# secondlaw-ai/skyrim

Measured on AMD Instinct MI355X. Metric: 6-h forecast steps/sec on 721x1440 state, 1/2/4/8 MI355X; per-channel max rel-err vs ref, higher is better.
Workload: dtype f16; 1 GPU; Pangu 6-h autoregressive rollout, 721x1440x69 state (13 levels x 5 vars + 4 surface), random-init weights (64 M params), state resident in HBM, 1 ensemble membe; parallelism=single GPU, members=1, finite=True, rounding=compensated, term_plan=0x66f

## Files before the change

skyrim_amd/csrc/api.hip:

```cpp
#include <cstdio>
#include <cstdlib>
#include <cstring>
#include <string>
#include <type_traits>
#include <vector>

#include "../../include/skyrim_pangu.h"
#include "launchers.h"

using namespace skp;

namespace {

constexpr int kDepths[4] = {2, 6, 6, 2};
constexpr int kBiasRows = 3312;

int pad_to(int n, int mult, int* front, int pad_mode) {
    const int padded = (n + mult - 1) / mult * mult;
    if (front) *front = pad_mode == SKPANGU_PAD_CENTRE ? (padded - n) / 2 : 0;
    return padded;
}

bool make_geom(const skpangu_config& c, Geom& g) {
    if (c.n_lat < 8 || c.n_lon <= 0 || c.n_lon % 96 != 0) return false;
// ... 127 lines not shown
        }
        prof_cat[prof_used] = cat;
        (void)hipEventRecord(prof_ev[prof_used], s);
        ++prof_used;
    }
    void profile(bool on) override { prof_on = on; prof_used = 0; }
    ~Engine() override { for (hipEvent_t e : prof_ev) (void)hipEventDestroy(e); }
    hipError_t profile_read(skpangu_stage_stat* out, int cap, int* n) override {
        static const char* names_split[C_COUNT] = {"embed", "qkv_r0", "attn_r0", "proj_r0", "fc1_r0", "fc2_r0", "qkv_r1", "attn_r1",
                                                   "proj_r1", "fc1_r1", "fc2_r1", "downsample", "upsample", "recover"};
        static const char* names_block[C_COUNT] = {"embed", "qkv_r0", "attn_r0", "proj_r0", "proj_mlp_r0", "fc2_r0", "qkv_r1", "attn_r1",
                                                   "proj_r1", "proj_mlp_r1", "fc2_r1", "downsample", "upsample", "recover"};
        const char* const* names = fused_block ? names_block : names_split;
        double ms[C_COUNT] = {0}; int cnt[C_COUNT] = {0};
        if (prof_used > 0) {
            hipError_t e = hipEventSynchronize(prof_ev[prof_used - 1]);
            if (e != hipSuccess) return e;
        }
        for (size_t i = 0; i + 1 < prof_used; ++i) {
            if (prof_cat[i] < 0) continue;
            float t = 0.f;
            hipError_t e = hipEventElapsedTime(&t, prof_ev[i], prof_ev[i + 1]);
            if (e != hipSuccess) return e;
            ms[prof_cat[i]] += t; cnt[prof_cat[i]]++;
        }
        const double sa = 2.0 * NPL, hw = (double)g.H1 * g.W1, NA_ = P::NA;
        double fl[C_COUNT], by[C_COUNT];
        for (int r = 0; r < 2; ++r) {
            const double C = r == 0 ? 192 : 384, mw = g.mwin[r], nt = g.ntok[r], heads = C / 32, wb = 2.0 * NW;
            const int o = r == 0 ? 0 : 5;
            fl[C_QKV0 + o] = 2 * mw * C * 3 * C;      by[C_QKV0 + o] = nt * C * 2 * NA_ + 3 * mw * C * 2 + 3 * C * C * wb;
            fl[C_ATTN0 + o] = g.nwin[r] * heads * 4.0 * 144 * 144 * 32;
            by[C_ATTN0 + o] = 3 * mw * C * 2 + mw * C * sa + (double)g.types[r] * heads * 3456 * 2;
            fl[C_PROJ0 + o] = 2 * mw * C * C;          by[C_PROJ0 + o] = mw * C * sa + 2 * nt * C * 4 + C * C * wb;
            fl[C_FC1_0 + o] = 2 * nt * C * 4 * C;      by[C_FC1_0 + o] = nt * C * 2 * NA_ + nt * 4 * C * sa + 4 * C * C * wb;
            fl[C_FC2_0 + o] = 2 * nt * C * 4 * C;      by[C_FC2_0 + o] = nt * 4 * C * sa + 2 * nt * C * 4 + 4 * C * C * wb;
            const int nblk = kDepths[r == 0 ? 0 : 1] + kDepths[r == 0 ? 3 : 2];
            const int nqa = r == 0 ? (qa_fused(0) ? kDepths[0] : 0) + (qa_fused(3) ? kDepths[3] : 0)
                                   : (qa_fused(1) ? kDepths[1] : 0) + (qa_fused(2) ? kDepths[2] : 0);
            if (nqa > 0) {
                const double qa_fl = fl[C_ATTN0 + o] + fl[C_QKV0 + o];
                const double qa_by = nt * C * 2 + mw * C * sa + 3 * C * C * wb + (double)g.types[r] * heads * 3456 * 2;
                fl[C_ATTN0 + o] = nqa == nblk ? qa_fl : (nqa * qa_fl + (nblk - nqa) * fl[C_ATTN0 + o]) / nblk;
                by[C_ATTN0 + o] = nqa == nblk ? qa_by : (nqa * qa_by + (nblk - nqa) * by[C_ATTN0 + o]) / nblk;
            }
            if (fused_block) {
                fl[C_FC1_0 + o] = 4 * nt * C * 4 * C;  by[C_FC1_0 + o] = 2 * nt * C * 4 + 8 * C * C * wb;
                fl[C_FC1_0 + o] += 2 * mw * C * C;     by[C_FC1_0 + o] += nt * C * sa + C * C * wb;
            }
        }
        fl[C_EMBED] = 2 * hw * 112 * 192 + 2 * 7 * hw * 160 * 192; by[C_EMBED] = (69.0 + 3) * g.n_lat * g.n_lon * 4 + g.ntok[0] * 192.0 * 4;
        fl[C_DOWN] = 2.0 * g.ntok[1] * 768 * 384;                   by[C_DOWN] = g.ntok[0] * 192.0 * 4 + g.ntok[1] * 384.0 * 4;
        fl[C_UP] = 2.0 * g.ntok[1] * 384 * 768 + 2.0 * g.ntok[0] * 192 * 192;
        by[C_UP] = g.ntok[1] * 384.0 * 4 + 2 * g.ntok[0] * 192.0 * sa + g.ntok[0] * 192.0 * 4;
        fl[C_RECOVER] = 2 * hw * 384 * 64 + 2 * 7 * hw * 384 * 160; by[C_RECOVER] = 2 * g.ntok[0] * 192.0 * 4 + 69.0 * g.n_lat * g.n_lon * 4;
        int k = 0;
        for (int c = 0; c < C_COUNT && k < cap; ++c, ++k) {
            std::memset(&out[k], 0, sizeof(out[k]));
            std::strncpy(out[k].name, names[c], sizeof(out[k].name) - 1);
            out[k].launches = cnt[c]; out[k].total_ms = ms[c]; out[k].flops = fl[c]; out[k].bytes = by[c];
        }
        *n = k;
        prof_used = 0;
        return hipSuccess;
    }

    LinW<T> take_lin(Arena& a, int N, int ldd) {
        LinW<T> l;
        const long long plane = (long long)N * ldd;
        l.w = a.take<T>((size_t)plane * NW);
        l.plane = plane; l.ldw = ldd;
        return l;
    }

    void plan_prepared(char* base) {
        Arena a{base, 0};
        w.mean = a.take<float>(69); w.std = a.take<float>(69); w.istd = a.take<float>(69);
        w.masks = a.take<float>((size_t)3 * g.n_lat * g.n_lon);
        w.embed_u = take_lin(a, 192, 160); w.embed_s = take_lin(a, 192, 128);
        w.embed_u_b = a.take<float>(192); w.embed_s_b = a.take<float>(192);
        int b = 0;
        for (int layer = 0; layer < 4; ++layer) {
            const int c = layer_dim(layer), heads = layer_heads(layer), res = layer_res(layer);
            for (int i = 0; i < kDepths[layer]; ++i, ++b) {
                BlockW<T>& bw = w.blk[b];
                bw.qkv = take_lin(a, 3 * c, c); bw.proj = take_lin(a, c, c);
                bw.fc1 = take_lin(a, 4 * c, c); bw.fc2 = take_lin(a, c, 4 * c);
                const bool t2 = two_term(layer);
                bw.w1f = fused_block && !t2 ? a.take<T>((size_t)8 * c * c) : nullptr;
                bw.w2f = fused_block && !t2 ? a.take<T>((size_t)8 * c * c) : nullptr;
                bw.projf = fused_block && !t2 ? a.take<T>((size_t)2 * c * c) : nullptr;
                bw.projh = t2 ? a.take<T>((size_t)c * c) : nullptr;
                bw.w1h = t2 ? a.take<T>((size_t)4 * c * c) : nullptr;
                bw.w2h = t2 ? a.take<T>((size_t)4 * c * c) : nullptr;
                bw.qkvf = rt_qkv && !qkv_one(layer) ? a.take<T>((size_t)6 * c * c) : nullptr;
                bw.qkvh = qkv_one(layer) ? a.take<T>((size_t)3 * c * c) : nullptr;
                bw.qkv_b = a.take<float>(3 * c); bw.proj_b = a.take<float>(c);
                bw.fc1_b = a.take<float>(4 * c); bw.fc2_b = a.take<float>(c);
                bw.n1_g = a.take<float>(c); bw.n1_b = a.take<float>(c);
                bw.n2_g = a.take<float>(c); bw.n2_b = a.take<float>(c);
                bias_elems[b] = (size_t)g.types[res] * heads * 3456;
                bw.bias_cmp = a.take<f16>(bias_elems[b]);
            }
        }
        w.down_g = a.take<float>(768); w.down_b = a.take<float>(768);
        w.down = take_lin(a, 384, 768);
        w.up1 = take_lin(a, 768, 384); w.up2 = take_lin(a, 192, 192);
        w.up_g = a.take<float>(192); w.up_b = a.take<float>(192);
        w.rec_u = take_lin(a, 160, 384); w.rec_s = take_lin(a, 64, 384);
        w.rec_u_b = a.take<float>(5); w.rec_s_b = a.take<float>(4);
        for (int r = 0; r < 2; ++r)
            for (int roll = 0; roll < 2; ++roll) { w.widx[r][roll] = a.take<int>(g.mwin[r]); w.winv[r][roll] = a.take<int>(g.ntok[r]); }
        zrow = a.take<T>(4096);
        qkv_w_tmp = a.take<float>((size_t)3 * 384 * 384); qkv_b_tmp = a.take<float>(3 * 384);
        cal_sum = a.take<float>(4 * 384);
        prep_bytes = (a.off + 255) / 256 * 256;
    }

    void plan_workspace(char* base) {
        Arena a{base, 0};
        const size_t n0 = (size_t)g.ntok[0] * 192, n1 = (size_t)g.ntok[1] * 384;
        wk.xs_plane[0] = (long long)n0; wk.xs_plane[1] = (long long)n1;
        wk.X1s = a.take<T>(n0 * 2); wk.X2s = a.take<T>(n1 * 2); wk.X4s = a.take<T>(n0 * 2);
        const size_t m0 = (size_t)g.mwin[0] * 192, m1 = (size_t)g.mwin[1] * 384;
        q_elems = m0 > m1 ? m0 : m1;
        wk.qkv_plane = (long long)q_elems;
        wk.q = a.take<f16>(q_elems); wk.k = a.take<f16>(q_elems); wk.vt = a.take<f16>(q_elems);
        ao_elems = q_elems;
        wk.ao_plane = (long long)ao_elems;
        wk.ao = a.take<T>(ao_elems * NPL);
        const size_t h0 = (size_t)g.ntok[0] * 768, h1 = (size_t)g.ntok[1] * 1536;
        hid_elems = h0 > h1 ? h0 : h1;
        wk.hid_plane = (long long)hid_elems;
        wk.hid = a.take<T>(hid_elems * NPL);
        wk.u_plane = (long long)n0;
        wk.u = a.take<T>(n0 * NPL);
        wk.stats = a.take<float2>((size_t)g.ntok[1]);
        ws_bytes = (a.off + 255) / 256 * 256;
    }

    explicit Engine(const Geom& geom, int qkv_a1 = 0, int mlp_mode = 0, int term_plan = 0) : g(geom) {
        fused_qa = getenv("SKP_SPLIT_ATTN") == nullptr;
        fused_block = mlp_mode == 0;
        rt_qkv = (std::is_same<P, PrecF16x3>::value && qkv_a1 && mlp_mode == 0);
        plan2 = (std::is_same<P, PrecF16x3>::value && fused_block) ? term_plan : 0;
        wk.qkv_a1 = qkv_a1;
        params = build_params(g, nullptr);
        plan_prepared(nullptr);
        plan_workspace(nullptr);
    }
    size_t prepared_bytes() const override { return prep_bytes; }
    size_t workspace_bytes() const override { return ws_bytes; }
    void bind(char* prepared, char* workspace) override { plan_prepared(prepared); plan_workspace(workspace); }

    const float* P_(const float* master, const std::string& name) const {
        for (const Param& p : params)
            if (p.name == name) return master + p.offset;
        return nullptr;
    }
    hipError_t copyf(const float* dst, const float* src, size_t n, hipStream_t s) {
        return hipMemcpyAsync(const_cast<float*>(dst), src, n * sizeof(float), hipMemcpyDeviceToDevice, s);
    }
    hipError_t lin(const LinW<T>& l, const float* src, int N, int K, long long sn, long long sk, hipStream_t s, int blocked = 1, int perm = 1) {
        return prep_weight<T, NW>(src, const_cast<T*>(l.w), l.plane, N, K, l.ldw, sn, sk, blocked, perm, s);
    }

#define CK(x) do { hipError_t e_ = (x); if (e_ != hipSuccess) return e_; } while (0)

    hipError_t prepare(const float* m, hipStream_t s) override {
        wk.zrow = zrow;
        CK(hipMemsetAsync(zrow, 0, 4096 * sizeof(T), s));
        CK(copyf(w.mean, P_(m, "norm.mean"), 69, s));
        CK(copyf(w.std, P_(m, "norm.std"), 69, s));
        CK(prep_reciprocal(P_(m, "norm.std"), const_cast<float*>(w.istd), 69, s));
        CK(copyf(w.masks, P_(m, "const_masks"), (size_t)3 * g.n_lat * g.n_lon, s));
        CK(lin(w.embed_u, P_(m, "embed.conv.weight"), 192, 160, 160, 1, s, 0));
        CK(lin(w.embed_s, P_(m, "embed.conv_surface.weight"), 192, 112, 112, 1, s, 0));
        CK(copyf(w.embed_u_b, P_(m, "embed.conv.bias"), 192, s));
        CK(copyf(w.embed_s_b, P_(m, "embed.conv_surface.bias"), 192, s));
        int b = 0;
        for (int layer = 0; layer < 4; ++layer) {
            const int c = layer_dim(layer), heads = layer_heads(layer), res = layer_res(layer);
            for (int i = 0; i < kDepths[layer]; ++i, ++b) {
                const std::string p = "layer" + std::to_string(layer + 1) + ".block" + std::to_string(i) + ".";
                const BlockW<T>& bw = w.blk[b];
                const float *qkv_w = P_(m, p + "attn.qkv.weight"), *qkv_bias = P_(m, p + "attn.qkv.bias");
                if (g.qkv_order) {
                    CK(prep_qkv_rows(qkv_w, qkv_bias, qkv_w_tmp, qkv_b_tmp, c, heads, s));
                    qkv_w = qkv_w_tmp; qkv_bias = qkv_b_tmp;
                }
                CK(lin(bw.qkv, qkv_w, 3 * c, c, c, 1, s));
                CK(lin(bw.proj, P_(m, p + "attn.proj.weight"), c, c, c, 1, s));
                CK(lin(bw.fc1, P_(m, p + "mlp.fc1.weight"), 4 * c, c, c, 1, s));
                CK(lin(bw.fc2, P_(m, p + "mlp.fc2.weight"), c, 4 * c, 4 * c, 1, s));
                if (bw.projf) CK(prep_rowtile_weights<T>(P_(m, p + "attn.proj.weight"), const_cast<T*>(bw.projf), c, c, s));
                if (bw.qkvf) CK(prep_rowtile_weights<T>(qkv_w, const_cast<T*>(bw.qkvf), 3 * c, c, s));
                if (bw.qkvh) CK(prep_rowtile_weights<T>(qkv_w, const_cast<T*>(bw.qkvh), 3 * c, c, s, 1));
                if (bw.w1f) CK(prep_mlp_weights<T>(P_(m, p + "mlp.fc1.weight"), P_(m, p + "mlp.fc2.weight"), const_cast<T*>(bw.w1f), const_cast<T*>(bw.w2f), c, s));
                if (bw.projh) {
                    CK(prep_rowtile_weights<T>(P_(m, p + "attn.proj.weight"), const_cast<T*>(bw.projh), c, c, s, 1));
                    CK(prep_mlp_weights<T>(P_(m, p + "mlp.fc1.weight"), P_(m, p + "mlp.fc2.weight"), const_cast<T*>(bw.w1h), const_cast<T*>(bw.w2h), c, s, 1));
                }
                CK(copyf(bw.qkv_b, qkv_bias, 3 * c, s));
                CK(copyf(bw.proj_b, P_(m, p + "attn.proj.bias"), c, s));
                CK(copyf(bw.fc1_b, P_(m, p + "mlp.fc1.bias"), 4 * c, s));
                CK(copyf(bw.fc2_b, P_(m, p + "mlp.fc2.bias"), c, s));
                CK(copyf(bw.n1_g, P_(m, p + "norm1.weight"), c, s));
                CK(copyf(bw.n1_b, P_(m, p + "norm1.bias"), c, s));
                CK(copyf(bw.n2_g, P_(m, p + "norm2.weight"), c, s));
                CK(copyf(bw.n2_b, P_(m, p + "norm2.bias"), c, s));
                CK(prep_bias_compact(P_(m, p + "attn.bias_table"), const_cast<f16*>(bw.bias_cmp), g.types[res], heads, g.nH[res], (i & 1) ? g.roll_sign : 0, g.mask_value, s, g.bias_transposed));
            }
        }
        CK(copyf(w.down_g, P_(m, "down.norm.weight"), 768, s));
        CK(copyf(w.down_b, P_(m, "down.norm.bias"), 768, s));
        CK(lin(w.down, P_(m, "down.linear.weight"), 384, 768, 768, 1, s, 0));
        CK(lin(w.up1, P_(m, "up.linear1.weight"), 768, 384, 384, 1, s));
        CK(lin(w.up2, P_(m, "up.linear2.weight"), 192, 192, 192, 1, s));
        CK(copyf(w.up_g, P_(m, "up.norm.weight"), 192, s));
        CK(copyf(w.up_b, P_(m, "up.norm.bias"), 192, s));
        CK(lin(w.rec_u, P_(m, "recover.conv.weight"), 160, 384, 1, 160, s, 1, 0));
        CK(lin(w.rec_s, P_(m, "recover.conv_surface.weight"), 64, 384, 1, 64, s, 1, 0));
        CK(copyf(w.rec_u_b, P_(m, "recover.conv.bias"), 5, s));
        CK(copyf(w.rec_s_b, P_(m, "recover.conv_surface.bias"), 4, s));
        const int H[2] = {g.H1, g.H2}, W[2] = {g.W1, g.W2};
        for (int r = 0; r < 2; ++r)
            for (int roll = 0; roll < 2; ++roll)
            {
                CK(prep_window_index(const_cast<int*>(w.widx[r][roll]), g.Z, H[r], W[r], g.Hp[r], g.top[r], roll ? g.roll_sign : 0, s, g.surface_last));
                CK(prep_window_inverse(w.widx[r][roll], g.mwin[r], const_cast<int*>(w.winv[r][roll]), s));
            }
        return hipSuccess;
    }

    static int block_index(int layer0, int i) {
        int b = 0;
        for (int l = 0; l < layer0; ++l) b += kDepths[l];
        return b + i;
    }

    hipError_t block_planes(int layer0, int i, T* xs, hipStream_t s) {
        const int res = layer_res(layer0), C = layer_dim(layer0), heads = layer_heads(layer0);
        const BlockW<T>& bw = w.blk[block_index(layer0, i)];
        const int* widx = w.widx[res][i & 1];
        const int o = res == 0 ? 0 : 5;
        bool fused = false;
        if constexpr (std::is_same<P, PrecF16x3>::value) {
            if (qa_fused(layer0)) {
                mark(C_ATTN0 + o, s);
                CK(op_qkv_attention(g, bw, widx, res, xs, wk, s, block_one(layer0) ? 1 : 2));
                fused = true;
            }
        }
        if (!fused) {
            mark(C_QKV0 + o, s);
            if constexpr (std::is_same<P, PrecF16x3>::value) {
                if (rt_qkv) CK(op_qkv_rowtile(g, bw, widx, res, xs, wk, s));
                else CK((op_qkv<P>(g, bw, widx, res, xs, wk, s)));
            } else {
                CK((op_qkv<P>(g, bw, widx, res, xs, wk, s)));
            }
            mark(C_ATTN0 + o, s);
            AttnArgs<P> a{wk.q, wk.k, wk.vt, bw.bias_cmp, wk.ao, wk.ao_plane, C, g.nwin[res], g.nW[res], heads};
            a.out_planes = block_one(layer0) ? 1 : 0;
            CK(launch_attention<P>(a, s));
        }
        if constexpr (std::is_same<P, PrecF16x3>::value) {
            if (two_term(layer0)) {
                mark(C_FC1_0 + o, s);
                CK(op_proj_mlp2(g, bw, w.winv[res][i & 1], res, xs, wk, s, block_one(layer0)));
                mark(-1, s);
// ... 91 lines not shown
            for (int i = 0; i < kDepths[layer]; ++i, ++b) {
                const int C = layer_dim(layer), heads = layer_heads(layer);
                const std::string p = "layer" + std::to_string(layer + 1) + ".block" + std::to_string(i) + ".";
                const BlockW<T>& bw = w.blk[b];
                const float *qkv_w = P_(m, p + "attn.qkv.weight"), *qkv_bias = P_(m, p + "attn.qkv.bias");
                if (g.qkv_order) { CK(prep_qkv_rows(qkv_w, qkv_bias, qkv_w_tmp, qkv_b_tmp, C, heads, s)); qkv_bias = qkv_b_tmp; }
                CK(copyf(bw.qkv_b, qkv_bias, 3 * C, s));
                CK(copyf(bw.proj_b, P_(m, p + "attn.proj.bias"), C, s));
                CK(copyf(bw.fc1_b, P_(m, p + "mlp.fc1.bias"), 4 * C, s));
                CK(copyf(bw.fc2_b, P_(m, p + "mlp.fc2.bias"), C, s));
            }
        return hipSuccess;
    }
    hipError_t calibrate(const float* m, const float* in, hipStream_t s) override {
        if (plan2 == 0) return hipSuccess;
        if (!in) return master_biases(m, s);
        if constexpr (std::is_same<P, PrecF16x3>::value) {
            CK((op_embed<P>(g, w, in, wk.X1s, wk, s)));
            for (int i = 0; i < kDepths[0]; ++i) CK(calib_block(m, 0, i, wk.X1s, s));
            CK((op_down<P>(g, w, wk.X1s, wk.X2s, wk, s)));
            for (int i = 0; i < kDepths[1]; ++i) CK(calib_block(m, 1, i, wk.X2s, s));
            for (int i = 0; i < kDepths[2]; ++i) CK(calib_block(m, 2, i, wk.X2s, s));
            CK((op_up<P>(g, w, wk.X2s, wk.X4s, wk, s)));
            for (int i = 0; i < kDepths[3]; ++i) CK(calib_block(m, 3, i, wk.X4s, s));
        }
        return hipSuccess;
    }

    hipError_t step(const float* in, float* out, hipStream_t s) override {
        mark(C_EMBED, s);
        CK((op_embed<P>(g, w, in, wk.X1s, wk, s)));
        for (int i = 0; i < kDepths[0]; ++i) CK(block_planes(0, i, wk.X1s, s));
        mark(C_DOWN, s);
        CK((op_down<P>(g, w, wk.X1s, wk.X2s, wk, s)));
        for (int i = 0; i < kDepths[1]; ++i) CK(block_planes(1, i, wk.X2s, s));
        for (int i = 0; i < kDepths[2]; ++i) CK(block_planes(2, i, wk.X2s, s));
        mark(C_UP, s);
        CK((op_up<P>(g, w, wk.X2s, wk.X4s, wk, s)));
        for (int i = 0; i < kDepths[3]; ++i) CK(block_planes(3, i, wk.X4s, s));
        mark(C_RECOVER, s);
        CK((op_recover<P>(g, w, wk.X1s, wk.X4s, out, wk, s)));
        mark(-1, s);
        return hipSuccess;
    }
#undef CK

    bool debug(const std::string& n, void** p, size_t* bytes) override {
        auto set = [&](const void* ptr, size_t b) { *p = const_cast<void*>(ptr); *bytes = b; return true; };
        if (n == "q") return set(wk.q, q_elems * sizeof(f16));
        if (n == "k") return set(wk.k, q_elems * sizeof(f16));
        if (n == "vt") return set(wk.vt, q_elems * sizeof(f16));
        if (n == "ao") return set(wk.ao, ao_elems * NPL * sizeof(T));
        if (n == "hid") return set(wk.hid, hid_elems * NPL * sizeof(T));
        if (n == "u") return set(wk.u, (size_t)g.ntok[0] * 192 * NPL * sizeof(T));
        if (n == "x1") return set(wk.X1s, (size_t)g.ntok[0] * 192 * 2 * sizeof(T));
        if (n == "x2") return set(wk.X2s, (size_t)g.ntok[1] * 384 * 2 * sizeof(T));
        if (n == "x4") return set(wk.X4s, (size_t)g.ntok[0] * 192 * 2 * sizeof(T));
        if (n.rfind("widx", 0) == 0 && n.size() == 6) {
            const int r = n[4] - '0', roll = n[5] - '0';
            if (r < 0 || r > 1 || roll < 0 || roll > 1) return false;
            return set(w.widx[r][roll], (size_t)g.mwin[r] * 4);
        }
        if (n.rfind("bias_exp", 0) == 0) {
            const int b = atoi(n.c_str() + 8);
            if (b < 0 || b > 15) return false;
            return set(w.blk[b].bias_cmp, bias_elems[b] * sizeof(f16));
        }
        return false;
    }
};

IEngine* make_engine(const skpangu_config& cfg, const Geom& g) {
    switch (cfg.precision) {
        case SKPANGU_PREC_BF16X3: return new Engine<PrecBF16x3>(g, 0, cfg.mlp_mode);
        case SKPANGU_PREC_F16X3: return new Engine<PrecF16x3>(g, 0, cfg.mlp_mode, cfg.term_plan);
        case SKPANGU_PREC_F16X3_Q: return new Engine<PrecF16x3>(g, 1, cfg.mlp_mode, cfg.term_plan);
        default: return nullptr;
    }
}

}

struct skpangu_ctx {
    skpangu_config cfg;
    Geom g;
    IEngine* eng;
    bool prepared;
};

extern "C" {

int skpangu_abi_version(void) { return SKPANGU_ABI_VERSION; }

const char* skpangu_error_string(int code) {
    switch (code) {
        case 0: return "success";
        case SKPANGU_E_ARG: return "bad argument or unsupported geometry";
        case SKPANGU_E_SIZE: return "caller buffer too small";
        case SKPANGU_E_STATE: return "context not prepared";
        case SKPANGU_E_NOTFOUND: return "not found";
        default: return code > 0 ? hipGetErrorString((hipError_t)code) : "unknown error";
    }
}

int skpangu_query_sizes(const skpangu_config* cfg, skpangu_sizes* out) {
    if (!cfg || !out) return SKPANGU_E_ARG;
    Geom g;
// ... 109 lines not shown
```

skyrim_amd/csrc/epilogues.h:

```cpp
#pragma once
#include "common.h"

namespace skp {

__device__ __forceinline__ void pin(f32x4& v) { asm volatile("" : "+v"(v)); }

__device__ __forceinline__ void add8(f32x4& lo, f32x4& hi, const float4& b0, const float4& b1) {
    lo[0] += b0.x; lo[1] += b0.y; lo[2] += b0.z; lo[3] += b0.w;
    hi[0] += b1.x; hi[1] += b1.y; hi[2] += b1.z; hi[3] += b1.w;
}

constexpr int kEpiReduceBytes = 4096;
constexpr int kEpiTableBytes = 8192;
constexpr int kEpiScratch = kEpiReduceBytes + kEpiTableBytes;


template <class T>
struct EpStorePlanes {
    static constexpr bool kDualOrder = false;
    template <class TC> __device__ __forceinline__ void init(char*, int, int) const {}
    const float* bias;
    int ld, row_off;
    T* out;
    long long plane;
// ... 86 lines not shown
#pragma unroll
                for (int a = 0; a < TC::FM; ++a) { add8(acc[a][2 * bp], acc[a][2 * bp + 1], b0, b1); pin(acc[a][2 * bp]); pin(acc[a][2 * bp + 1]); }
            }
#pragma unroll
            for (int a = 0; a < TC::FM; ++a) {
                const int m = m0w + a * 16 + l15;
                if (m >= M) continue;
                const int win = m / WIN_TOKENS, t = m - win * WIN_TOKENS;
#pragma unroll
                for (int bp = 0; bp < TC::FN / 2; ++bp) {
                    const int n = n0w + bp * 32 + l8;
                    if (n >= N) continue;
                    const int which = n >= C ? 1 : 0;
                    const int c = n - which * C;
                    const int head = c >> 5, d = c & 31;
                    const float s = which == 0 ? scale : 1.0f;
                    const f32x4 &x = acc[a][2 * bp], &y = acc[a][2 * bp + 1];
                    const float v[8] = {x[0] * s, x[1] * s, x[2] * s, x[3] * s, y[0] * s, y[1] * s, y[2] * s, y[3] * s};
                    T* dst = (which == 0 ? q : k) + (((long long)win * heads + head) * WIN_TOKENS + t) * HEAD_DIM + d;
                    store8_planes<T, NPL>(dst, plane, v);
                }
            }
        } else {
#pragma unroll
            for (int b = 0; b < TC::FN; ++b) {
                const int n = perm8_col(n0w + b * 16 + l15);
                const float bb = bias[n < N ? n : 0];
#pragma unroll
                for (int a = 0; a < TC::FM; ++a) { acc[a][b][0] += bb; acc[a][b][1] += bb; acc[a][b][2] += bb; acc[a][b][3] += bb; pin(acc[a][b]); }
            }
#pragma unroll
            for (int ap = 0; ap < TC::FM / 2; ++ap) {
                const int m = m0w + ap * 32 + 2 * l4;
                if (m >= M) continue;
                const int win = m / WIN_TOKENS, t = m - win * WIN_TOKENS;
#pragma unroll
                for (int b = 0; b < TC::FN; ++b) {
                    const int n = perm8_col(n0w + b * 16 + l15);
                    if (n >= N) continue;
                    const int c = n - 2 * C;
                    const int head = c >> 5, d = c & 31;
                    const f32x4 &x = acc[2 * ap][b], &y = acc[2 * ap + 1][b];
                    const float v[8] = {x[0], x[1], x[2], x[3], y[0], y[1], y[2], y[3]};
                    store8_planes<T, NPL>(vt + (((long long)win * heads + head) * HEAD_DIM + d) * WIN_TOKENS + t, plane, v);
                }
            }
        }
    }
};

struct RowMapIndexed {
    const int* idx;
    __device__ __forceinline__ long long dest(int m, int) const { return idx ? idx[m] : m; }
};
struct RowMapPixelShuffle {
    int H1, W1, H2, W2;
    __device__ __forceinline__ long long dest(int m, int ntile) const {
        const int hw = H2 * W2;
        const int z = m / hw, rem = m - z * hw;
        const int h = rem / W2, w = rem - h * W2;
        const int hf = 2 * h + (ntile >> 1), wf = 2 * w + (ntile & 1);
        if (hf >= H1 || wf >= W1) return -1;
        return ((long long)z * H1 + hf) * W1 + wf;
    }
};
struct f32x8 { float4 a, b; };
template <class T>
struct SinkResidual {
    T* xs;
    long long plane;
    static constexpr bool kLoads = true;
    __device__ __forceinline__ f32x8 load(long long row, int ld, int c) const {
        const T* p = xs + blk_off(row, c, ld);
        const typename OpT<T>::v8 h = as_v8<T>(*reinterpret_cast<const uint4*>(p));
        const typename OpT<T>::v8 l = as_v8<T>(*reinterpret_cast<const uint4*>(p + plane));
        f32x8 o;
        o.a = make_float4((float)h[0] + (float)l[0], (float)h[1] + (float)l[1], (float)h[2] + (float)l[2], (float)h[3] + (float)l[3]);
        o.b = make_float4((float)h[4] + (float)l[4], (float)h[5] + (float)l[5], (float)h[6] + (float)l[6], (float)h[7] + (float)l[7]);
        return o;
    }
    __device__ __forceinline__ void put(long long row, int ld, int c, const float (&y)[8], const f32x8& old) const {
        const float v[8] = {old.a.x + y[0], old.a.y + y[1], old.a.z + y[2], old.a.w + y[3],
                            old.b.x + y[4], old.b.y + y[5], old.b.z + y[6], old.b.w + y[7]};
        store8_planes<T, 2>(xs + blk_off(row, c, ld), plane, v);
    }
};
template <class T, int NPL>
struct SinkStore {
    T* out;
    long long plane;
    static constexpr bool kLoads = false;
    __device__ __forceinline__ f32x8 load(long long, int, int) const { return f32x8{}; }
    __device__ __forceinline__ void put(long long row, int ld, int c, const float (&y)[8], const f32x8&) const {
        store8_planes<T, NPL>(out + blk_off(row, c, ld), plane, y);
    }
};

template <class RowMap, class Sink, int GROUP = 1>
struct EpLayerNorm {
    static constexpr bool kDualOrder = false;
    template <class TC> __device__ __forceinline__ void init(char* tab, int tid, int n0) const {
        float* t = reinterpret_cast<float*>(tab);
        for (int i = tid; i < TC::BN; i += TC::THREADS) {
            t[i] = gamma[i];
            t[TC::BN + i] = beta[i];
            t[2 * TC::BN + i] = bias != nullptr ? bias[n0 + i] : 0.f;
        }
    }
    RowMap map;
    Sink sink;
    const float* bias;
    const float* gamma;
    const float* beta;
    float eps;
    int n_groups = 0;
    template <class TC, bool SWAP>
    __device__ __forceinline__ void run(f32x4 (&acc)[TC::FM][TC::FN], int m0w, int n0w, int lane, int wm, int wn, char* smem, int M, int N, int ntile) const {
        static_assert(SWAP && TC::FN % 2 == 0, "swapped order, fragment pairs");
        static_assert(GROUP == 1 || (GROUP == TC::FM && !Sink::kLoads), "grouped rows: one member per fragment, no residual");
        constexpr int FM = TC::FM, FN = TC::FN, FP = TC::FN / 2, WN = TC::WN, BM = TC::BM, BN = TC::BN;
        const int l15 = lane & 15, l8 = (lane >> 4) * 8;
        const int nloc0 = n0w - ntile * BN;
        float* red = reinterpret_cast<float*>(smem);
        const float* tab = reinterpret_cast<const float*>(smem + kEpiReduceBytes);
        static_assert(3 * BN * 4 <= kEpiTableBytes && 2 * BM * WN * 4 <= kEpiReduceBytes, "epilogue LDS scratch");
#pragma unroll
        for (int bp = 0; bp < FP; ++bp) {
            const float* bsrc = tab + 2 * BN + nloc0 + bp * 32 + l8;
            const float4 b0 = *reinterpret_cast<const float4*>(bsrc), b1 = *reinterpret_cast<const float4*>(bsrc + 4);
#pragma unroll
            for (int a = 0; a < FM; ++a) add8(acc[a][2 * bp], acc[a][2 * bp + 1], b0, b1);
        }
        long long drow[FM];
        bool ok[FM];
#pragma unroll
        for (int a = 0; a < FM; ++a) {
            const int m = m0w + a * 16 + l15;
            const long long r = map.dest(m < M ? m : 0, ntile);
            ok[a] = m < M && r >= 0;
            drow[a] = ok[a] ? r : 0;
        }
        constexpr int PRE = FM < 3 ? FM : 3;
        f32x8 old[Sink::kLoads ? FM : 1][Sink::kLoads ? FP : 1];
        if constexpr (Sink::kLoads) {
#pragma unroll
            for (int a = 0; a < PRE; ++a)
#pragma unroll
                for (int bp = 0; bp < FP; ++bp) old[a][bp] = sink.load(drow[a], BN, nloc0 + bp * 32 + l8);
        }
// ... 133 lines not shown
```

skyrim_amd/csrc/launchers.h:

```cpp
#pragma once
#include <hip/hip_runtime.h>
#include "common.h"

namespace skp {

struct Geom {
    int n_lat, n_lon, n_levels, n_channels, surf0;
    int lat_top;
    int Z, H1, W1, H2, W2;
    int Hp[2], top[2], nH[2], nW[2], types[2], nwin[2];
    int ntok[2], mwin[2];
    int roll_sign;
    float mask_value;
    int surface_last, qkv_order, bias_transposed;
};

template <class T>
struct LinW { const T* w; long long plane; int ldw; };

template <class T>
struct BlockW {
    LinW<T> qkv, proj, fc1, fc2;
    const T *w1f, *w2f;
    const T *projf, *qkvf;
    const T *projh, *w1h, *w2h;
    const T* qkvh;
    const float *qkv_b, *proj_b, *fc1_b, *fc2_b, *n1_g, *n1_b, *n2_g, *n2_b;
    const f16* bias_cmp;
};

template <class T>
struct ModelW {
    const float *mean, *std, *istd, *masks;
    LinW<T> embed_u, embed_s;
    const float *embed_u_b, *embed_s_b;
    BlockW<T> blk[16];
    const float *down_g, *down_b;
    LinW<T> down;
    LinW<T> up1, up2;
    const float *up_g, *up_b;
    LinW<T> rec_u, rec_s;
    const float *rec_u_b, *rec_s_b;
    const int* widx[2][2];
    const int* winv[2][2];
};

template <class P>
struct Work {
    typedef typename P::T T;
    T *X1s, *X2s, *X4s;
    long long xs_plane[2];
    f16 *q, *k, *vt;
    long long qkv_plane;
    T *ao, *hid, *u;
    long long ao_plane, hid_plane, u_plane;
    const T* zrow;
    int qkv_a1;
    float2* stats;
};

template <class P>
struct AttnArgs {
    const f16 *q, *k, *vt;
    const f16* bias_cmp;
    typename P::T* out;
    long long out_plane;
    int ld_out, n_win, nW, heads;
    int out_planes = 0;
};

inline int layer_res(int layer) { return (layer == 0 || layer == 3) ? 0 : 1; }
inline int layer_dim(int layer) { return layer_res(layer) == 0 ? 192 : 384; }
inline int layer_heads(int layer) { return layer_res(layer) == 0 ? 6 : 12; }

template <class P> hipError_t launch_attention(const AttnArgs<P>&, hipStream_t);

template <class P> hipError_t op_embed(const Geom&, const ModelW<typename P::T>&, const float* state, typename P::T* X1s, const Work<P>&, hipStream_t);
template <class P> hipError_t op_recover(const Geom&, const ModelW<typename P::T>&, const typename P::T* skip_s, const typename P::T* x4_s, float* state, const Work<P>&, hipStream_t);
template <class P> hipError_t op_qkv(const Geom&, const BlockW<typename P::T>&, const int* widx, int res, const typename P::T* Xs, const Work<P>&, hipStream_t);
template <class P> hipError_t op_proj(const Geom&, const BlockW<typename P::T>&, const int* widx, int res, typename P::T* Xs, const Work<P>&, hipStream_t);
template <class P> hipError_t op_fc1(const Geom&, const BlockW<typename P::T>&, int res, const typename P::T* Xs, const Work<P>&, hipStream_t);
template <class P> hipError_t op_fc2(const Geom&, const BlockW<typename P::T>&, int res, typename P::T* Xs, const Work<P>&, hipStream_t);
template <class P> hipError_t op_down(const Geom&, const ModelW<typename P::T>&, const typename P::T* X1s, typename P::T* X2s, const Work<P>&, hipStream_t);
template <class P> hipError_t op_up(const Geom&, const ModelW<typename P::T>&, const typename P::T* X2s, typename P::T* X4s, const Work<P>&, hipStream_t);
template <class T> hipError_t prep_mlp_weights(const float* w1, const float* w2, T* w1f, T* w2f, int C, hipStream_t, int planes = 2);
hipError_t op_qkv_rowtile(const Geom&, const BlockW<f16>&, const int* widx, int res, const f16* Xs, const Work<PrecF16x3>&, hipStream_t);
template <class T> hipError_t prep_rowtile_weights(const float* w, T* wf, int N, int K, hipStream_t, int planes = 2);
hipError_t op_qkv_attention(const Geom&, const BlockW<f16>&, const int* widx, int res, const f16* Xs, const Work<PrecF16x3>&, hipStream_t, int out_planes);
template <class P> hipError_t op_proj_mlp_fused(const Geom&, const BlockW<typename P::T>&, const int* winv, int res, typename P::T* Xs, const Work<P>&, hipStream_t);
hipError_t op_proj_mlp2(const Geom&, const BlockW<f16>&, const int* winv, int res, f16* Xs, const Work<PrecF16x3>&, hipStream_t, int one = 0);
template <class T, int NPL> hipError_t split_planes(const float* x, T* planes, long long plane, long long n, int C, hipStream_t);
template <class T> hipError_t merge_planes(const T* planes, long long plane, float* x, long long n, int C, hipStream_t);

template <class T, int NW>
hipError_t prep_weight(const float* src, T* dst, long long plane, int N, int K, int ldd, long long sn, long long sk, int blocked, int perm, hipStream_t);
hipError_t prep_bias_compact(const float* table, f16* out, int types, int heads, int nH, int roll, float mask_value, hipStream_t, int transposed = 0);
hipError_t prep_qkv_rows(const float* w, const float* b, float* w_out, float* b_out, int C, int heads, hipStream_t);
hipError_t prep_window_index(int* idx, int Z, int H, int W, int Hp, int top, int roll, hipStream_t, int surface_last = 0);
hipError_t prep_window_inverse(const int* idx, int n, int* inv, hipStream_t);
hipError_t prep_reciprocal(const float* src, float* dst, int n, hipStream_t);
template <class T> hipError_t colsum_planes(const T* x, long long plane, int nplanes, const int* rowmap, int rows, int K, float* scratch, float* out, hipStream_t);
size_t colsum_scratch_floats(int rows, int K);
hipError_t bias_fold(const float* w, const float* colsum, float scale, float* bias, int N, int K, hipStream_t);
template <class T> hipError_t merge_stats(const T* x, long long plane, float2* stats, int Z, int H1, int W1, int H2, int W2, int C, float eps, hipStream_t);

inline bool aligned16(const void* p) { return (reinterpret_cast<size_t>(p) & 15) == 0; }

inline int hip_status(int e_hip) { return hipGetLastError() == hipSuccess ? 0 : e_hip; }
// ... 10 lines not shown
```

skyrim_amd/csrc/ops_updown.hip:

```cpp
#include "tiles.h"

namespace skp {

template <class P>
hipError_t op_down(const Geom& g, const ModelW<typename P::T>& w, const typename P::T* X1s, typename P::T* X2s, const Work<P>& wk, hipStream_t s) {
    typedef typename P::T T;
    typedef EpStorePlanes<T> EP;
    SKP_CHECK((merge_stats<T>(X1s, wk.xs_plane[0], wk.stats, g.Z, g.H1, g.W1, g.H2, g.W2, 192, 1e-5f, s)));
    GemmArgs<P, ALMergeLN<T>, EP> a;
    a.al = ALMergeLN<T>{X1s, wk.xs_plane[0], wk.stats, w.down_g, w.down_b, g.H1, g.W1, g.H2, g.W2, 192, g.ntok[1]};
    a.ep = EP{nullptr, 384, 0, X2s, wk.xs_plane[1]};
    a.W = w.down.w; a.w_plane = w.down.plane; a.ldw = w.down.ldw;
    a.M = g.ntok[1]; a.N = 384; a.K = 768;
    return launch_gemm<P, typename Tiles<P>::D384>(a, s);
}

template <class P>
hipError_t op_up(const Geom& g, const ModelW<typename P::T>& w, const typename P::T* X2s, typename P::T* X4s, const Work<P>& wk, hipStream_t s) {
    typedef typename P::T T;
    typedef typename Tiles<P>::D192 TC;
    {
        typedef EpLayerNorm<RowMapPixelShuffle, SinkStore<T, P::NA>> EP;
        DmaArgs<P, APlanes<T>, EP> a;
        a.as = APlanes<T>{X2s, wk.xs_plane[1], 384, nullptr, g.ntok[1]};
        a.ep = EP{RowMapPixelShuffle{g.H1, g.W1, g.H2, g.W2}, SinkStore<T, P::NA>{wk.u, wk.u_plane}, nullptr, w.up_g, w.up_b, 1e-5f};
        a.W = w.up1.w; a.w_plane = w.up1.plane; a.ldw = w.up1.ldw; a.zrow = wk.zrow;
        a.M = g.ntok[1]; a.N = 768; a.K = 384;
        SKP_CHECK((launch_gemm_dma<P, TC>(a, s)));
    }
    {
        typedef EpStorePlanes<T> EP;
        DmaArgs<P, APlanes<T>, EP> a;
        a.as = APlanes<T>{wk.u, wk.u_plane, 192, nullptr, g.ntok[0]};
        a.ep = EP{nullptr, 192, 0, X4s, wk.xs_plane[0]};
        a.W = w.up2.w; a.w_plane = w.up2.plane; a.ldw = w.up2.ldw; a.zrow = wk.zrow;
        a.M = g.ntok[0]; a.N = 192; a.K = 192;
        SKP_CHECK((launch_gemm_dma<P, TC>(a, s)));
    }
    return hipSuccess;
}

template hipError_t op_down<PrecBF16x3>(const Geom&, const ModelW<bf16>&, const bf16*, bf16*, const Work<PrecBF16x3>&, hipStream_t);
template hipError_t op_down<PrecF16x3>(const Geom&, const ModelW<f16>&, const f16*, f16*, const Work<PrecF16x3>&, hipStream_t);
template hipError_t op_up<PrecBF16x3>(const Geom&, const ModelW<bf16>&, const bf16*, bf16*, const Work<PrecBF16x3>&, hipStream_t);
template hipError_t op_up<PrecF16x3>(const Geom&, const ModelW<f16>&, const f16*, f16*, const Work<PrecF16x3>&, hipStream_t);

}
```

Baseline: 75.46 steps/s.

## Fuse up-sample linear1, LayerNorm and linear2 into one kernel

Replaces the two-GEMM up-sampling path with a single kernel. It computes linear1 per pixel-shuffle quadrant, applies LayerNorm in registers, then runs linear2 and writes the shuffled output directly. This drops the intermediate u buffer and its HBM round trip, plus one launch. The cost is serialized weight streaming through double-buffered LDS with full barriers per chunk, and weights re-streamed for every block.

Result: no change. 76.04 steps/s (median of 3 runs) (+0.8%).

```diff
diff --git a/skyrim_amd/csrc/api.hip b/skyrim_amd/csrc/api.hip
--- a/skyrim_amd/csrc/api.hip
+++ b/skyrim_amd/csrc/api.hip
@@ -203,7 +203,7 @@
         fl[C_EMBED] = 2 * hw * 112 * 192 + 2 * 7 * hw * 160 * 192; by[C_EMBED] = (69.0 + 3) * g.n_lat * g.n_lon * 4 + g.ntok[0] * 192.0 * 4;
         fl[C_DOWN] = 2.0 * g.ntok[1] * 768 * 384;                   by[C_DOWN] = g.ntok[0] * 192.0 * 4 + g.ntok[1] * 384.0 * 4;
         fl[C_UP] = 2.0 * g.ntok[1] * 384 * 768 + 2.0 * g.ntok[0] * 192 * 192;
-        by[C_UP] = g.ntok[1] * 384.0 * 4 + 2 * g.ntok[0] * 192.0 * sa + g.ntok[0] * 192.0 * 4;
+        by[C_UP] = g.ntok[1] * 384.0 * 4 + g.ntok[0] * 192.0 * 4 + (768.0 * 384 + 192.0 * 192) * 2 * NW;
         fl[C_RECOVER] = 2 * hw * 384 * 64 + 2 * 7 * hw * 384 * 160; by[C_RECOVER] = 2 * g.ntok[0] * 192.0 * 4 + 69.0 * g.n_lat * g.n_lon * 4;
         int k = 0;
         for (int c = 0; c < C_COUNT && k < cap; ++c, ++k) {
@@ -256,7 +256,7 @@
         }
         w.down_g = a.take<float>(768); w.down_b = a.take<float>(768);
         w.down = take_lin(a, 384, 768);
-        w.up1 = take_lin(a, 768, 384); w.up2 = take_lin(a, 192, 192);
+        w.up1f = a.take<T>((size_t)2 * 768 * 384); w.up2f = a.take<T>((size_t)2 * 192 * 192);
         w.up_g = a.take<float>(192); w.up_b = a.take<float>(192);
         w.rec_u = take_lin(a, 160, 384); w.rec_s = take_lin(a, 64, 384);
         w.rec_u_b = a.take<float>(5); w.rec_s_b = a.take<float>(4);
@@ -284,8 +284,6 @@
         hid_elems = h0 > h1 ? h0 : h1;
         wk.hid_plane = (long long)hid_elems;
         wk.hid = a.take<T>(hid_elems * NPL);
-        wk.u_plane = (long long)n0;
-        wk.u = a.take<T>(n0 * NPL);
         wk.stats = a.take<float2>((size_t)g.ntok[1]);
         ws_bytes = (a.off + 255) / 256 * 256;
     }
@@ -366,8 +364,8 @@
         CK(copyf(w.down_g, P_(m, "down.norm.weight"), 768, s));
         CK(copyf(w.down_b, P_(m, "down.norm.bias"), 768, s));
         CK(lin(w.down, P_(m, "down.linear.weight"), 384, 768, 768, 1, s, 0));
-        CK(lin(w.up1, P_(m, "up.linear1.weight"), 768, 384, 384, 1, s));
-        CK(lin(w.up2, P_(m, "up.linear2.weight"), 192, 192, 192, 1, s));
+        CK(prep_rowtile_weights<T>(P_(m, "up.linear1.weight"), const_cast<T*>(w.up1f), 768, 384, s));
+        CK(prep_rowtile_weights<T>(P_(m, "up.linear2.weight"), const_cast<T*>(w.up2f), 192, 192, s));
         CK(copyf(w.up_g, P_(m, "up.norm.weight"), 192, s));
         CK(copyf(w.up_b, P_(m, "up.norm.bias"), 192, s));
         CK(lin(w.rec_u, P_(m, "recover.conv.weight"), 160, 384, 1, 160, s, 1, 0));
@@ -565,7 +563,6 @@
         if (n == "vt") return set(wk.vt, q_elems * sizeof(f16));
         if (n == "ao") return set(wk.ao, ao_elems * NPL * sizeof(T));
         if (n == "hid") return set(wk.hid, hid_elems * NPL * sizeof(T));
-        if (n == "u") return set(wk.u, (size_t)g.ntok[0] * 192 * NPL * sizeof(T));
         if (n == "x1") return set(wk.X1s, (size_t)g.ntok[0] * 192 * 2 * sizeof(T));
         if (n == "x2") return set(wk.X2s, (size_t)g.ntok[1] * 384 * 2 * sizeof(T));
         if (n == "x4") return set(wk.X4s, (size_t)g.ntok[0] * 192 * 2 * sizeof(T));
diff --git a/skyrim_amd/csrc/epilogues.h b/skyrim_amd/csrc/epilogues.h
--- a/skyrim_amd/csrc/epilogues.h
+++ b/skyrim_amd/csrc/epilogues.h
@@ -162,17 +162,6 @@
 struct RowMapIndexed {
     const int* idx;
     __device__ __forceinline__ long long dest(int m, int) const { return idx ? idx[m] : m; }
-};
-struct RowMapPixelShuffle {
-    int H1, W1, H2, W2;
-    __device__ __forceinline__ long long dest(int m, int ntile) const {
-        const int hw = H2 * W2;
-        const int z = m / hw, rem = m - z * hw;
-        const int h = rem / W2, w = rem - h * W2;
-        const int hf = 2 * h + (ntile >> 1), wf = 2 * w + (ntile & 1);
-        if (hf >= H1 || wf >= W1) return -1;
-        return ((long long)z * H1 + hf) * W1 + wf;
-    }
 };
 struct f32x8 { float4 a, b; };
 template <class T>
@@ -195,16 +184,6 @@
         store8_planes<T, 2>(xs + blk_off(row, c, ld), plane, v);
     }
 };
-template <class T, int NPL>
-struct SinkStore {
-    T* out;
-    long long plane;
-    static constexpr bool kLoads = false;
-    __device__ __forceinline__ f32x8 load(long long, int, int) const { return f32x8{}; }
-    __device__ __forceinline__ void put(long long row, int ld, int c, const float (&y)[8], const f32x8&) const {
-        store8_planes<T, NPL>(out + blk_off(row, c, ld), plane, y);
-    }
-};
 
 template <class RowMap, class Sink, int GROUP = 1>
 struct EpLayerNorm {
diff --git a/skyrim_amd/csrc/launchers.h b/skyrim_amd/csrc/launchers.h
--- a/skyrim_amd/csrc/launchers.h
+++ b/skyrim_amd/csrc/launchers.h
@@ -37,7 +37,7 @@
     BlockW<T> blk[16];
     const float *down_g, *down_b;
     LinW<T> down;
-    LinW<T> up1, up2;
+    const T *up1f, *up2f;
     const float *up_g, *up_b;
     LinW<T> rec_u, rec_s;
     const float *rec_u_b, *rec_s_b;
@@ -52,8 +52,8 @@
     long long xs_plane[2];
     f16 *q, *k, *vt;
     long long qkv_plane;
-    T *ao, *hid, *u;
-    long long ao_plane, hid_plane, u_plane;
+    T *ao, *hid;
+    long long ao_plane, hid_plane;
     const T* zrow;
     int qkv_a1;
     float2* stats;
diff --git a/skyrim_amd/csrc/ops_updown.hip b/skyrim_amd/csrc/ops_updown.hip
--- a/skyrim_amd/csrc/ops_updown.hip
+++ b/skyrim_amd/csrc/ops_updown.hip
@@ -1,3 +1,6 @@
+#include <type_traits>
+#include "blockrow.h"
+#include "launchers.h"
 #include "tiles.h"
 
 namespace skp {
@@ -15,29 +18,164 @@
     return launch_gemm<P, typename Tiles<P>::D384>(a, s);
 }
 
+template <class T>
+struct UpArgs {
+    const T* x; long long x_plane;
+    int M;
+    T* out; long long out_plane;
+    const T *w1f, *w2f;
+    const float *gamma, *beta;
+    int H1, W1, H2, W2;
+    float eps;
+};
+
+struct UpShape {
+    static constexpr int CIN = 384, C = 192, KS1 = CIN / 32, KS2 = C / 32, CF = C / 16, NB = C / 32, NWAVES = 8, THREADS = 64 * NWAVES, BM = NWAVES * 16;
+    static constexpr int BLK1 = KS1 * 2 * 2, BLK2 = KS2 * 2 * 2;
+    static constexpr int STAGE = BLK1 * 1024;
+    static constexpr int SMEM = 2 * STAGE + 2 * C * 4;
+    static_assert(BLK1 % NWAVES == 0 && BLK2 % NWAVES == 0 && NB % 2 == 0, "whole DMA pieces per wave; every group starts in stage 0");
+};
+
+template <class T>
+__global__ void __launch_bounds__(UpShape::THREADS) __attribute__((amdgpu_waves_per_eu(2, 2)))
+upsample_kernel(const UpArgs<T> a) {
+    typedef UpShape S;
+    constexpr int C = S::C, KS1 = S::KS1, KS2 = S::KS2, CF = S::CF, NB = S::NB, NWAVES = S::NWAVES, RD = 3;
+    typedef typename OpT<T>::v8 v8;
+    extern __shared__ __attribute__((aligned(16))) char smem[];
+    float* tab = reinterpret_cast<float*>(smem + 2 * S::STAGE);
+    const int tid = threadIdx.x, lane = tid & 63, l15 = lane & 15, g = lane >> 4;
+    const int wave = __builtin_amdgcn_readfirstlane(tid >> 6);
+    const unsigned lds_base = (unsigned)(size_t)smem;
+    char* st0 = smem;
+    char* st1 = smem + S::STAGE;
+
+    auto dma = [&](const T* src_blocks, unsigned dst, auto nkib) {
+#pragma unroll
+        for (int i = 0; i < decltype(nkib)::value / NWAVES; ++i) {
+            const int b = wave + i * NWAVES;
+            glds16_s(src_blocks + (b << 9), (unsigned)lane * 16, dst + (unsigned)(b << 10));
+        }
+    };
+    const std::integral_constant<int, S::BLK1> kib1;
+    const std::integral_constant<int, S::BLK2> kib2;
+    dma(a.w1f, lds_base, kib1);
+    for (int i = tid; i < C; i += S::THREADS) { tab[i] = a.gamma[i]; tab[C + i] = a.beta[i]; }
+
+    const long long rb = (long long)blockIdx.x * NWAVES + wave;
+    const bool live = rb * 16 < a.M;
+    v8 xh[KS1], xl[KS1];
+    {
+        const T* p = a.x + ((live ? rb : 0) * KS1 << 9) + l15 * 32 + g * 8;
+#pragma unroll
+        for (int ks = 0; ks < KS1; ++ks) {
+            xh[ks] = *reinterpret_cast<const v8*>(p + (ks << 9));
+            xl[ks] = *reinterpret_cast<const v8*>(p + (ks << 9) + a.x_plane);
+        }
+#pragma unroll
+        for (int ks = 0; ks < KS1; ++ks) asm volatile("" : "+v"(xh[ks]), "+v"(xl[ks]));
+    }
+    const int m = (int)(live ? rb : 0) * 16 + l15;
+    const int hw = a.H2 * a.W2;
+    const int z = m / hw, rem = m - z * hw;
+    const int h = rem / a.W2, w = rem - h * a.W2;
+
+    for (int q = 0; q < 4; ++q) {
+        f32x4 acc[CF];
+#pragma unroll
+        for (int c = 0; c < CF; ++c) acc[c] = f32x4{0.f, 0.f, 0.f, 0.f};
+#pragma unroll
+        for (int j = 0; j < NB; ++j) {
+            asm volatile("s_waitcnt vmcnt(0)" ::: "memory");
+            __syncthreads();
+            if (j + 1 < NB) dma(a.w1f + ((long long)(q * NB + j + 1) * S::BLK1 << 9), lds_base + (unsigned)(((j + 1) & 1) * S::STAGE), kib1);
+            else dma(a.w2f, lds_base, kib2);
+            sk_stream<KS1 * 2, RD>(((j & 1) ? st1 : st0) + lane * 16, [&](int s, const uint4& wh, const uint4& wl) {
+                const int ks = s >> 1, c = 2 * j + (s & 1);
+                acc[c] = OpT<T>::mfma(as_v8<T>(wl), xh[ks], acc[c]);
+                acc[c] = OpT<T>::mfma(as_v8<T>(wh), xl[ks], acc[c]);
+                acc[c] = OpT<T>::mfma(as_v8<T>(wh), xh[ks], acc[c]);
+            });
+        }
+
+        v8 uh[KS2], ul[KS2];
+        {
+            float s = 0.f;
+#pragma unroll
+            for (int bp = 0; bp < KS2; ++bp)
+#pragma unroll
+                for (int r = 0; r < 4; ++r) s += acc[2 * bp][r] + acc[2 * bp + 1][r];
+            s += __shfl_xor(s, 16);
+            s += __shfl_xor(s, 32);
+            const float mean = s * (1.0f / C);
+            float v2 = 0.f;
+#pragma unroll
+            for (int c = 0; c < CF; ++c)
+#pragma unroll
+                for (int r = 0; r < 4; ++r) { const float d = acc[c][r] - mean; v2 += d * d; }
+            v2 += __shfl_xor(v2, 16);
+            v2 += __shfl_xor(v2, 32);
+            const float rstd = rsqrtf(v2 * (1.0f / C) + a.eps);
+#pragma unroll
+            for (int bp = 0; bp < KS2; ++bp) {
+                const int n = 32 * bp + 8 * g;
+                const float4 g0 = *reinterpret_cast<const float4*>(tab + n), g1 = *reinterpret_cast<const float4*>(tab + n + 4);
+                const float4 e0 = *reinterpret_cast<const float4*>(tab + C + n), e1 = *reinterpret_cast<const float4*>(tab + C + n + 4);
+                const f32x4 &x = acc[2 * bp], &y = acc[2 * bp + 1];
+                const float v[8] = {(x[0] - mean) * rstd * g0.x + e0.x, (x[1] - mean) * rstd * g0.y + e0.y, (x[2] - mean) * rstd * g0.z + e0.z, (x[3] - mean) * rstd * g0.w + e0.w,
+                                    (y[0] - mean) * rstd * g1.x + e1.x, (y[1] - mean) * rstd * g1.y + e1.y, (y[2] - mean) * rstd * g1.z + e1.z, (y[3] - mean) * rstd * g1.w + e1.w};
+                uint4 o[2];
+                split8<T, 2>(v, o);
+                uh[bp] = as_v8<T>(o[0]);
+                ul[bp] = as_v8<T>(o[1]);
+            }
+        }
+
+        f32x4 out[CF];
+#pragma unroll
+        for (int c = 0; c < CF; ++c) out[c] = f32x4{0.f, 0.f, 0.f, 0.f};
+#pragma unroll
+        for (int j = 0; j < NB; ++j) {
+            asm volatile("s_waitcnt vmcnt(0)" ::: "memory");
+            __syncthreads();
+            if (j + 1 < NB) dma(a.w2f + ((long long)(j + 1) * S::BLK2 << 9), lds_base + (unsigned)(((j + 1) & 1) * S::STAGE), kib2);
+            else if (q + 1 < 4) dma(a.w1f + ((long long)(q + 1) * NB * S::BLK1 << 9), lds_base, kib1);
+            sk_stream<KS2 * 2, RD>(((j & 1) ? st1 : st0) + lane * 16, [&](int s, const uint4& wh, const uint4& wl) {
+                const int ks = s >> 1, c = 2 * j + (s & 1);
+                out[c] = OpT<T>::mfma(as_v8<T>(wl), uh[ks], out[c]);
+                out[c] = OpT<T>::mfma(as_v8<T>(wh), ul[ks], out[c]);
+                out[c] = OpT<T>::mfma(as_v8<T>(wh), uh[ks], out[c]);
+            });
+        }
+
+        const int hf = 2 * h + (q >> 1), wf = 2 * w + (q & 1);
+        if (live && hf < a.H1 && wf < a.W1) {
+            const long long tf = ((long long)z * a.H1 + hf) * a.W1 + wf;
+            T* dst = a.out + blk_off(tf, g * 8, C);
+#pragma unroll
+            for (int bp = 0; bp < KS2; ++bp) {
+                const f32x4 &x = out[2 * bp], &y = out[2 * bp + 1];
+                const float v[8] = {x[0], x[1], x[2], x[3], y[0], y[1], y[2], y[3]};
+                store8_planes<T, 2>(dst + (bp << 9), a.out_plane, v);
+            }
+        }
+    }
+}
+
 template <class P>
 hipError_t op_up(const Geom& g, const ModelW<typename P::T>& w, const typename P::T* X2s, typename P::T* X4s, const Work<P>& wk, hipStream_t s) {
     typedef typename P::T T;
-    typedef typename Tiles<P>::D192 TC;
-    {
-        typedef EpLayerNorm<RowMapPixelShuffle, SinkStore<T, P::NA>> EP;
-        DmaArgs<P, APlanes<T>, EP> a;
-        a.as = APlanes<T>{X2s, wk.xs_plane[1], 384, nullptr, g.ntok[1]};
-        a.ep = EP{RowMapPixelShuffle{g.H1, g.W1, g.H2, g.W2}, SinkStore<T, P::NA>{wk.u, wk.u_plane}, nullptr, w.up_g, w.up_b, 1e-5f};
-        a.W = w.up1.w; a.w_plane = w.up1.plane; a.ldw = w.up1.ldw; a.zrow = wk.zrow;
-        a.M = g.ntok[1]; a.N = 768; a.K = 384;
-        SKP_CHECK((launch_gemm_dma<P, TC>(a, s)));
-    }
-    {
-        typedef EpStorePlanes<T> EP;
-        DmaArgs<P, APlanes<T>, EP> a;
-        a.as = APlanes<T>{wk.u, wk.u_plane, 192, nullptr, g.ntok[0]};
-        a.ep = EP{nullptr, 192, 0, X4s, wk.xs_plane[0]};
-        a.W = w.up2.w; a.w_plane = w.up2.plane; a.ldw = w.up2.ldw; a.zrow = wk.zrow;
-        a.M = g.ntok[0]; a.N = 192; a.K = 192;
-        SKP_CHECK((launch_gemm_dma<P, TC>(a, s)));
-    }
-    return hipSuccess;
+    typedef UpShape S;
+    static_assert(P::NA == 2 && P::NW == 2, "three terms");
+    UpArgs<T> a{X2s, wk.xs_plane[1], g.ntok[1], X4s, wk.xs_plane[0], w.up1f, w.up2f, w.up_g, w.up_b, g.H1, g.W1, g.H2, g.W2, 1e-5f};
+    if (a.M % 16 != 0) return hipErrorInvalidValue;
+    auto kern = upsample_kernel<T>;
+    SKP_CHECK(hipFuncSetAttribute(reinterpret_cast<const void*>(kern), hipFuncAttributeMaxDynamicSharedMemorySize, S::SMEM));
+    const unsigned grid = (unsigned)((a.M + S::BM - 1) / S::BM);
+    if (grid == 0) return hipSuccess;
+    hipLaunchKernelGGL(kern, dim3(grid), dim3(S::THREADS), S::SMEM, s, a);
+    return hipGetLastError();
 }
 
 template hipError_t op_down<PrecBF16x3>(const Geom&, const ModelW<bf16>&, const bf16*, bf16*, const Work<PrecBF16x3>&, hipStream_t);
```
